# microsoft/ConfigNet

Measured on AMD Instinct MI355X. Metric: train-step images/sec at 256x256 (G+D fwd+bwd), higher is better.
Workload: dtype f32; 1 GPU; ConfigNet second-stage iteration (D + synth-D + latent-D + G + EMA), 256x256, batch 16 per GPU, fp32, Keras-Adam; global_batch=16, resolution=256, latent_dim=145, parallelism=dp1, losses_finite=True

## Files before the change

### confignet_amd/_lib.py

```python
import ctypes
import os

_HERE = os.path.dirname(os.path.abspath(__file__))
LIB_PATH = os.environ.get("CN_LIB") or os.path.join(_HERE, "libconfignet_hip.so")


class CnSumJob(ctypes.Structure):
    _fields_ = [("src", ctypes.c_void_p), ("dst", ctypes.c_void_p), ("count", ctypes.c_longlong), ("parts", ctypes.c_int),
                ("accumulate", ctypes.c_int)]


class CnDepthJob(ctypes.Structure):
    _fields_ = [("a", ctypes.c_void_p), ("b", ctypes.c_void_p), ("c", ctypes.c_void_p), ("m", ctypes.c_int), ("n", ctypes.c_int),
                ("k", ctypes.c_int), ("lda", ctypes.c_int), ("ldb", ctypes.c_int), ("ldc", ctypes.c_int)]


class CnRowsJob(ctypes.Structure):
    _fields_ = [("a", ctypes.c_void_p), ("b", ctypes.c_void_p), ("c", ctypes.c_void_p), ("bias", ctypes.c_void_p), ("mask", ctypes.c_void_p)] + \
               [(n_, ctypes.c_int) for n_ in ("m", "n", "k", "lda", "ldb", "ldc", "tb", "act", "accumulate")] + [("slope", ctypes.c_float)]


class CnGanJob(ctypes.Structure):
    _fields_ = [("s", ctypes.c_void_p), ("out", ctypes.c_void_p), ("gout", ctypes.c_void_p), ("n", ctypes.c_int), ("label", ctypes.c_float)]

# ... 56 lines not shown
    "cn_gemm_rows_grouped": [_p, _i, _p],
    "cn_gemm_rows_grouped_k": [_p, _i, _p],
    "cn_gemm_rows_grouped_plan": [_p, _i, ctypes.POINTER(_i), _i, ctypes.POINTER(_i)],
    "cn_conv_tune": [_i, _i, ctypes.c_long],
    "cn_conv_fwd_plan": [_G, _i, _i, _i, _i, _i, _i, _i, ctypes.POINTER(ctypes.c_int * 8)],
    "cn_conv_fwd_plan_ep": [_G, _i, _i, _i, _i, _i, _i, _i, _i, ctypes.POINTER(ctypes.c_int * 8)],
    "cn_conv_loop_select": [_i, _i, _i, _i],
    "cn_fwd2_col_block": [_i, _i, _i, _i, _i, _i],
    "cn_conv_fwd_dt": [_p, _p, _i, _p, _p, _p, _i, _i, _f, _p],
    "cn_conv_dgrad_dt": [_p, _p, _i, _p, _p, _i, _p],
    "cn_conv_wgrad_c3_partials": [],
    "cn_conv_wgrad_c3": [_p, _p, _p, _i, _p, _p, _i, _p],
    "cn_conv_wino_filter": [_p, _p, _i, _i, _i, _p],
    "cn_conv_fwd_wino": [_i, _i, _i, _i, _i, _p, _p, _p, _p, _i, _f, _p],
    "cn_conv_fwd_wino_ep": [_i, _i, _i, _i, _i, _p, _p, _p, _p, _p, _p, _p],
    "cn_conv_fwd_wino4": [_i, _i, _i, _i, _i, _p, _p, _p, _p, _i, _f, _p],
    "cn_conv_fwd_wino4_ep": [_i, _i, _i, _i, _i, _p, _p, _p, _p, _i, _f, _i, _p, _p, _p, _p, _i, _f, _p],
    "cn_conv_wino4_filter": [_p, _p, _i, _i, _i, _p],
    "cn_sumpool2": [_p, _p, _i, _i, _i, _i, _i, _i, _i, _p],
    "cn_gemm": [_i, _i, _i, _i, _i, _p, _i, _p, _i, _p, _i, _p, _i, _f, _p],
    "cn_gemm_plan": [_i] * 10 + [ctypes.POINTER(ctypes.c_int * 9)],
    "cn_nc_reduce4": [_p, _p, _i, _i, _i, _f, _i, _i, _p],
    "cn_nc_reduce": [_p, _p, _p, _p, _i, _i, _i, _i, _f, _i, _p],
    "cn_nc_reduce_plan": [_i, _i, _i, _i, _i, _i, ctypes.POINTER(ctypes.c_int * 8)],
    "cn_nc_lin2": [_p, _p, _p, _p, _p, _p, _p, _p, _i, _i, _i, _i, _i, _f, _i, _p],
    "cn_nc_rows_plan": [ctypes.c_longlong, _i, _i, ctypes.POINTER(ctypes.c_int * 2)],
    "cn_norm_coef_fwd": [_i, _p, _p, _p, _p, _p, _p, _p, _p, _i, _i, _i, _f, _p, _i, _p],
    "cn_norm_coef_bwd": [_i, _p, _p, _p, _p, _p, _p, _p, _p, _p, _p, _i, _i, _i, _f, _p],
    "cn_dual_tail_coef_fwd": [_p] * 13 + [_i, _i, _i, _f, _i, _i, _p],
    "cn_dual_tail_coef_bwd": [_p] * 13 + [ctypes.POINTER(ctypes.c_void_p), _i, _i, _i, _f, _i, _i, _p],
    "cn_dual_tail_gx": [_p] * 12 + [_i, _i, _i, _f, _i, _i, _p],
    "cn_dual_tail_gx_tx": [_p] * 18 + [_i, _i, _i, _f, _i, _i, _i, _p],
    "cn_norm_apply": [_i, _i] + [_p] * 13 + [_i, _i, _i, _f, _i, _f, _i, _p],
    "cn_nc_reduce_hxt": [_p, _p, _p, _p, _i, _i, _i, _f, _i, _i, _i, _p],
    "cn_zero": [_p, ctypes.c_size_t, _p],
    "cn_set_deterministic": [_i],
    "cn_get_deterministic": [],
    "cn_det_release_stream": [_p],
    "cn_gemm_acc": [_i, _i, _i, _i, _i, _p, _i, _p, _i, _p, _i, _p],
    "cn_sum_rows_into": [_p, _p, _i, _i, _i, _p],
    "cn_bn_act_bwd": [_p, _p, _p, _p, _p, _p, _p, _p, _i, _i, _i, _i, _i, _i, _p],
    "cn_nc_reduce_dact": [_p, _p, _p, _p, _p, _i, _i, _i, _i, _f, _i, _i, _p],
    "cn_act_fwd": [_p, _p, _z, _i, _f, _i, _p],
    "cn_act_bwd": [_p, _p, _p, _z, _i, _f, _i, _p],
    "cn_act_bwd_bias": [_p, _p, _p, _p, _i, _i, _i, _i, _f, _i, _i, _p],
    "cn_axpby": [_p, _p, _p, _z, _f, _f, _i, _p],
    "cn_mul": [_p, _p, _p, _z, _i, _p],
    "cn_sqdiff_sum": [_p, _p, _p, _z, _f, _i, _p],
    "cn_row_sumsq": [_p, _p, _i, _z, _p],
    "cn_row_scale": [_p, _p, _p, _i, _z, _f, _i, _p],
    "cn_row_scale_diff": [_p, _p, _p, _p, _i, ctypes.c_size_t, _f, _i, _p],
    "cn_tap_bwd": [_p, _p, _p, _p, _p, _i, ctypes.c_size_t, _f, _i, _f, _i, _p],
    "cn_maxpool2_bwd_act": [_p, _p, _p, _p, _f, _p, _i, _i, _i, _i, _i, _i, _p],
    "cn_stream_plan": [_i, _i, ctypes.c_longlong, _z, _i, _i, _i, _i, _i, _i, ctypes.c_uint, _i, ctypes.POINTER(ctypes.c_longlong * 4)],
    "cn_stream_plan_ptrs": [_i, _i, _i, ctypes.c_longlong, _z, _i, _i, _i, _i, _i, _i, ctypes.POINTER(ctypes.c_void_p * 4), _i, ctypes.POINTER(ctypes.c_longlong * 4)],
    "cn_stream_last_plan": [ctypes.POINTER(ctypes.c_longlong * 5)],
    "cn_masked_diff": [_p, _p, _p, _p, _z, _i, _p],
    "cn_maxpool_fwd": [_p, _p, _i, _i, _i, _i, _i, _i, _i, _i, _p],
    "cn_maxpool_bwd": [_p, _p, _p, _i, _i, _i, _i, _i, _i, _i, _i, _p],
    "cn_avgpool3_same": [_p, _p, _i, _i, _i, _i, _i, _p],
    "cn_dwconv3x3_fwd": [_p, _p, _p, _p, _i, _i, _i, _i, _i, _i, _f, _p],
    "cn_image_preprocess": [_p, _i, _p, _i, _i, _i, _i, _i, _i, _f, _f, _p],
    "cn_dwconv3x3_dgrad": [_p, _p, _p, _i, _i, _i, _i, _i, _p],
    "cn_dwconv3x3_wgrad_slices": [_i, _i, _i, _i, _i],
    "cn_dwconv3x3_wgrad": [_p, _p, _p, _i, _i, _i, _i, _i, _i, _p],
    "cn_bn_train_coef": [_p] * 12 + [ctypes.c_longlong, _i, _f, ctypes.c_double, _i, _p],
# ... 51 lines not shown
```

### confignet_amd/csrc/elementwise.hip

```cpp
#include "common.h"
#include "typed.h"
#include <stdlib.h>

namespace {

__device__ __forceinline__ float lrelu(float v, float s) { return v > 0.f ? v : v * s; }


template <int V> struct RowV { float v[V]; };

template <int V, typename T>
__device__ __forceinline__ RowV<V> ld_row(const T* p) {
    RowV<V> r;
    if constexpr (V == 4) {
        const float4 t = ld4<T>(p);
        r.v[0] = t.x; r.v[1] = t.y; r.v[2] = t.z; r.v[3] = t.w;
    } else {
        r.v[0] = ldf<T>(p);
    }
    return r;
}
template <int V, typename T>
__device__ __forceinline__ void st_row(T* p, const RowV<V>& r) {
    if constexpr (V == 4) st4<T>(p, make_float4(r.v[0], r.v[1], r.v[2], r.v[3]));
// ... 1208 lines not shown
    }
    CN_DISPATCH_DT(dt, {
        if (V == 4) hipLaunchKernelGGL((nc_lin2_kernel<4, T>), dim3(ew_blocks(total)), dim3(256), 0, st, (const T*)x1, a1, (const T*)x2, a2, bb, a3, b3, (T*)y, total, s, c, cstride, flags, slope, period2);
        else hipLaunchKernelGGL((nc_lin2_kernel<1, T>), dim3(ew_blocks(total)), dim3(256), 0, st, (const T*)x1, a1, (const T*)x2, a2, bb, a3, b3, (T*)y, total, s, c, cstride, flags, slope, period2);
    });
    CN_LAUNCH_CHECK();
    return CN_OK;
}

extern "C" int cn_norm_apply(int mode, int dir, const void* x1, const void* x2, const float* sa, const float* sb, const float* p1,
                             const float* p2, float* save_mean, float* save_r, float* gp1, float* gp2, const float* a3,
                             const float* b3, void* y, int n, int s, int c, float eps, int flags, float slope, int dt, void* stream) {
    CN_CHECK_ARG((mode == 0 || mode == 1) && (dir == 0 || dir == 1) && x1 && sa && sb && p1 && save_mean && save_r && y && n > 0 && s > 0 && c > 0 &&
                 (dt == CN_F32 || dt == CN_BF16), "norm_apply: bad args");
    CN_CHECK_ARG(mode == 0 || dir == 1 || p2, "norm_apply: instance norm needs beta");
    CN_CHECK_ARG(dir == 0 || (x2 && gp1 && (mode == 0 || gp2)), "norm_apply: backward needs x and the parameter gradients' tensors");
    if (c % 4 != 0) return CN_EUNSUPPORTED;
    const int period2 = flags >> 8;
    CN_CHECK_ARG(period2 == 0 || (x2 && n % period2 == 0), "norm_apply: bad x2 period %d for n = %d", period2, n);
    flags &= 255;
    const int CG = c / 4;
    const long G = (long)s * CG;
    const NcRowsPlan rp = plan_nc_rows(G, CG, n);
    if (!rp.rows || (long)rp.gx * 256 < CG) return CN_EUNSUPPORTED;
    NormApplyArgs A;
    A.mode = mode; A.dir = dir; A.N = n; A.C = c; A.invS = 1.f / (float)s; A.eps = eps;
    A.s1 = sa; A.s2 = sb; A.p1 = p1; A.p2 = p2; A.sm = save_mean; A.sr = save_r; A.gp1 = gp1; A.gp2 = gp2;
    CN_DISPATCH_DT(dt, hipLaunchKernelGGL((norm_apply_rows_kernel<T>), dim3(rp.gx, n), dim3(256), 0, (hipStream_t)stream, A, (const T*)x1,
                                          (const T*)x2, a3, b3, (T*)y, (int)G, CG, flags, slope, period2));
    CN_LAUNCH_CHECK();
    return CN_OK;
}

#define EW_LAUNCH(kernel, n, ...)                                                                              \
    hipLaunchKernelGGL(kernel, dim3(ew_blocks(n)), dim3(256), 0, (hipStream_t)stream, __VA_ARGS__);             \
    CN_LAUNCH_CHECK();                                                                                         \
    return CN_OK;

static inline bool alv(const void* p, int dt) { return ((uintptr_t)p & (dt == CN_BF16 ? 7 : 15)) == 0; }
struct StreamPtrs { const void* p[4]; };
static inline unsigned stream_mask(int op, int dt, int dst_dt, const StreamPtrs& o) {
    unsigned m = 0;
    for (int i = 0; i < SP_OPERANDS[op]; ++i)
        if (alv(o.p[i], op == SP_CAST && i == 1 ? dst_dt : dt)) m |= 1u << i;
    return m;
}
static inline StreamReq stream_req(int op, int dt, long rows, size_t row) {
    return StreamReq{op, dt, rows, row, 0, 0, 0, 0, 0, 0, 0u, cn_det()};
}
static inline StreamReq pool_req(int op, int dt, int n, int h, int w, int c, int k, int s, int pad) {
    return StreamReq{op, dt, n, 0, c, h, w, k, s, pad, 0u, cn_det()};
}
static thread_local long long g_stream_last[5] = {-1, 0, 0, 0, 0};
static inline int stream_entry_plan(StreamReq r, int dst_dt, const StreamPtrs& o, StreamPlan* sp) {
    r.aligned = stream_mask(r.op, r.dt, dst_dt, o);
    const int e = plan_stream(r, sp);
    g_stream_last[0] = e ? -1 : r.op; g_stream_last[1] = sp->path; g_stream_last[2] = sp->gx; g_stream_last[3] = sp->gy; g_stream_last[4] = sp->parts;
    return e;
}
#define EW_LAUNCH_VT(kernel, op, n, ptrs, dt, ...)                                                                                \
    CN_CHECK_ARG((dt) == CN_F32 || (dt) == CN_BF16, "bad dtype code %d", (int)(dt));                                                \
    StreamPlan sp;                                                                                                                \
    if (int e__ = stream_entry_plan(stream_req(op, dt, 1, n), dt, ptrs, &sp)) return e__;                                         \
    CN_DISPATCH_DT(dt, {                                                                                                          \
        if (sp.path == SP_VEC) hipLaunchKernelGGL((kernel<true, T>), dim3(sp.gx), dim3(256), 0, (hipStream_t)stream, __VA_ARGS__); \
        else hipLaunchKernelGGL((kernel<false, T>), dim3(sp.gx), dim3(256), 0, (hipStream_t)stream, __VA_ARGS__);                  \
    });                                                                                                                           \
// ... 437 lines not shown
```

### confignet_amd/functional.py

```python
import contextlib

import torch
from torch.autograd import Function

from . import ops
from .ops import ACT_LRELU, ACT_NONE, ACT_RELU, ACT_TANH, ConvSpec

_INPUT_GRADS_ONLY = False
FUSED_TAIL_STATS = True
FUSED_R1_TAIL = True
BN_BWD_FUSED = True


@contextlib.contextmanager
def input_grads_only():
    global _INPUT_GRADS_ONLY
    prev, _INPUT_GRADS_ONLY = _INPUT_GRADS_ONLY, True
    try:
        yield
    finally:
        _INPUT_GRADS_ONLY = prev


class _RefuseFn(Function):
# ... 416 lines not shown
        if x1 is not None and ctx.needs_input_grad[0]:
            gx1 = NcLinFn.apply(gy, a1, None, None, None, pc)
        if a1 is not None and ctx.needs_input_grad[1]:
            sum_gy, ga1 = NcSumDotFn.apply(gy, x1, pc)
        if x2 is not None and ctx.needs_input_grad[2]:
            gx2 = NcLinFn.apply(gy, a2, None, None, None, pc)
        if a2 is not None and ctx.needs_input_grad[3]:
            sum_gy2, ga2 = NcSumDotFn.apply(gy, x2, pc)
            sum_gy = sum_gy if sum_gy is not None else sum_gy2
        if need_b:
            gb = sum_gy if sum_gy is not None else NcSumDotFn.apply(gy, None, pc)[0]
        return gx1, ga1, gx2, ga2, gb, None, None


def nc_stats(x, per_channel=False):
    return NcSumDotFn.apply(x, None, per_channel)


def nc_lin(x1, a1=None, x2=None, a2=None, b=None, per_channel=False):
    return NcLinFn.apply(x1, a1, x2, a2, b, per_channel)


def _spatial(x):
    return x.numel() // (x.shape[0] * x.shape[-1])


class AdaInFn(Function):

    @staticmethod
    def forward(ctx, x, scale_bias):
        x, sb = _cg(x), _cg(scale_bias)
        sp = _spatial(x)
        st = ops.take_stats(x, "act")
        s1, s2 = st if st is not None else ops.nc_reduce(x)
        fused = ops.norm_apply_fwd(ops.NORM_ADAIN, x, s1, s2, sb, None, 1e-3)
        if fused is not None:
            y, mean, r = fused
            ctx.save_for_backward(x, sb, mean, r)
            return y
        a, b, mean, r = ops.norm_coef_fwd(ops.NORM_ADAIN, s1, s2, sb, None, sp, 1e-3, x)
        ctx.save_for_backward(x, sb, mean, r)
        return ops.nc_lin2(tuple(x.shape), x, a, b=b)

    @staticmethod
    def backward(ctx, gy):
        if torch.is_grad_enabled():
            raise RuntimeError("AdaInFn is first-order only; use adain_composite()")
        x, sb, mean, r = ctx.saved_tensors
        gy = _cg(gy)
        t1, t2 = ops.nc_reduce(gy, x)
        fused = ops.norm_apply_bwd(ops.NORM_ADAIN, gy, x, t1, t2, mean, r, sb, 1e-3)
        if fused is not None:
            return fused[0], fused[1]
        c1, c2, c0, gsb, _ = ops.norm_coef_bwd(ops.NORM_ADAIN, t1, t2, mean, r, sb, _spatial(x), 1e-3)
        return ops.nc_lin2(tuple(x.shape), gy, c1, x, c2, c0), gsb


def adain(x, scale_bias):
    return AdaInFn.apply(x, scale_bias)


def adain_composite(x, scale_bias):
    c = x.shape[-1]
    s_, b_ = scale_bias[:, :c], scale_bias[:, c:]
    inv = 1.0 / _spatial(x)
    s1, s2 = nc_stats(x)
    mu = s1 * inv
    var = s2 * inv - mu * mu
    a = torch.rsqrt(var + 1e-3) * (s_ + 1.0)
    return nc_lin(x, a, None, None, b_ - mu * a)


class DiscrTailFn(Function):

    @staticmethod
    def forward(ctx, x, gamma, beta, want_style, slope):
        ctx.set_materialize_grads(False)
        x, gamma, beta = _cg(x), _cg(gamma), _cg(beta)
        sp = _spatial(x)
        style = smean = ssd = None
        st = ops.take_stats(x, "pre4")
        if st is not None:
            s1, s2, a1, a2 = st
            if want_style:
                style, _, smean, ssd = ops.norm_coef_fwd(ops.NORM_STYLE, s1, s2, None, None, sp, 1e-6)
        elif want_style and FUSED_TAIL_STATS and x.shape[-1] % 4 == 0:
            s1, s2, a1, a2 = ops.nc_reduce4(x, slope)
            style, _, smean, ssd = ops.norm_coef_fwd(ops.NORM_STYLE, s1, s2, None, None, sp, 1e-6)
        else:
            if want_style:
                s1, s2 = ops.nc_reduce(x)
                style, _, smean, ssd = ops.norm_coef_fwd(ops.NORM_STYLE, s1, s2, None, None, sp, 1e-6)
            a1, a2 = ops.nc_reduce(x, flags=1, slope=slope)
        fused = ops.norm_apply_fwd(ops.NORM_INSTANCE, x, a1, a2, gamma, beta, 1e-3, flags=1, slope=slope)
        if fused is not None:
            y, mean, q = fused
        else:
            a, b, mean, q = ops.norm_coef_fwd(ops.NORM_INSTANCE, a1, a2, gamma, beta, sp, 1e-3)
            y = ops.nc_lin2(tuple(x.shape), x, a, b=b, flags=1, slope=slope)
        ctx.save_for_backward(x, gamma, mean, q, smean, ssd)
        ctx.slope, ctx.want_style = slope, want_style
        nd = [t for t in (mean, q, smean, ssd) if t is not None]
        ctx.mark_non_differentiable(*nd)
        return y, style, mean, q, smean, ssd

    @staticmethod
    def backward(ctx, gy, gstyle, *_):
        if torch.is_grad_enabled():
            raise RuntimeError("DiscrTailFn is first-order only; use the composite discr_block path")
        x, gamma, mean, q, smean, ssd = ctx.saved_tensors
        sp = _spatial(x)
        have_y = gy is not None
        d2 = d0 = None
        if ctx.want_style and gstyle is not None:
            _, d2, d0, _, _ = ops.norm_coef_bwd(ops.NORM_STYLE, _cg(gstyle), None, smean, ssd, None, sp, 1e-6)
        if have_y:
            gy = _cg(gy)
            t1, t2 = ops.nc_reduce(gy, x, flags=2, slope=ctx.slope)
            fused = ops.norm_apply_bwd(ops.NORM_INSTANCE, gy, x, t1, t2, mean, q, gamma, 1e-3, flags=2 | 4, slope=ctx.slope, a3=d2, b3=d0)
            if fused is not None:
                return fused[0], fused[1], fused[2], None, None
            c1, c2, c0, ggamma, gbeta = ops.norm_coef_bwd(ops.NORM_INSTANCE, t1, t2, mean, q, gamma, sp, 1e-3)
            gx = ops.nc_lin2(tuple(x.shape), gy, c1, x, c2, c0, flags=2 | 4, slope=ctx.slope, a3=d2, b3=d0)
            return gx, ggamma, gbeta, None, None
        gx = ops.nc_lin2(tuple(x.shape), x, d2, b=d0) if d2 is not None else torch.zeros_like(x)
        return gx, torch.zeros_like(gamma), torch.zeros_like(gamma), None, None


class DualTailFn(Function):

    @staticmethod
    def forward(ctx, tx, x, gamma, mean, q, smean, ssd, want_ty, want_style, slope):
        ctx.set_materialize_grads(False)
        tx, x = _cg(tx), _cg(x)
        sp = _spatial(x)
        shape = tuple(x.shape)
        ta = T = U = None
        if want_ty:
            ta = ops.act_bwd(tx, x, ACT_LRELU, slope)
            T = ops.nc_reduce(ta, x, flags=2, slope=slope)
        if want_style:
            U = ops.nc_reduce(tx, x)
        C1, C2, C0, tstyle = ops.dual_tail_coef_fwd(T, U, mean if want_ty else None, q if want_ty else None,
                                                    smean if want_style else None, ssd if want_style else None,
                                                    gamma, sp)
        ty = ops.nc_lin2(shape, ta, C1, x, C2, C0, flags=2, slope=slope) if want_ty else None
        ctx.save_for_backward(tx, x, gamma, mean, q, smean, ssd, ta,
                              T[0] if T else None, T[1] if T else None, U[0] if U else None, U[1] if U else None)
        ctx.cfg = (want_ty, want_style, slope)
        return ty, tstyle

    @staticmethod
    def backward(ctx, h, u):
        if torch.is_grad_enabled():
            raise RuntimeError("DualTailFn is first-order only")
        tx, x, gamma, mean, q, smean, ssd, ta, T1, T2, U1, U2 = ctx.saved_tensors
        want_ty, want_style, slope = ctx.cfg
# ... 357 lines not shown
```

### confignet_amd/ops.py

```python
import contextlib
import ctypes
import math
import os
import threading

import torch

from ._lib import CN_BF16, CN_EUNSUPPORTED, CN_F32, CN_U8, CnConvGeom, CnDepthJob, CnGanJob, CnRowsJob, CnSumJob, check, lib

ACT_NONE, ACT_LRELU, ACT_RELU, ACT_TANH, ACT_RELU6, ACT_SIGMOID = 0, 1, 2, 3, 4, 5

ACT_DTYPE = torch.float32


def set_activation_dtype(dtype):
    global ACT_DTYPE
    if isinstance(dtype, str):
        dtype = {"f32": torch.float32, "fp32": torch.float32, "float32": torch.float32, "bf16": torch.bfloat16,
                 "bfloat16": torch.bfloat16}[dtype]
    assert dtype in (torch.float32, torch.bfloat16)
    ACT_DTYPE = dtype


def _stream():
# ... 944 lines not shown
    n, s, c = _nsc(x)
    y = torch.empty_like(x)
    mean = torch.empty((n, c), device=x.device, dtype=torch.float32)
    r = torch.empty_like(mean)
    rc = lib.cn_norm_apply(mode, 0, _ptr(x), None, _fptr(s1), _fptr(s2), _fptr(_c(p1)), _fptr(None if p2 is None else _c(p2)), _ptr(mean), _ptr(r),
                           None, None, None, None, _ptr(y), n, s, c, eps, flags, slope, _dt(x), _stream())
    if rc == CN_EUNSUPPORTED:
        return None
    check(rc, "cn_norm_apply")
    return y, mean, r


def norm_apply_bwd(mode, gy, x, t1, t2, mean, r, p1, eps, flags=0, slope=0.0, a3=None, b3=None):
    if not NORM_APPLY or x.shape[-1] % 4 or x.dtype != torch.float32 or gy.dtype != torch.float32:
        return None
    gy, x = _unify(gy, x)
    n, s, c = _nsc(x)
    if flags & 4:
        _log_mask(x)
    gx = torch.empty_like(x)
    if mode == NORM_ADAIN:
        gp1, gp2 = torch.empty((n, 2 * c), device=x.device, dtype=torch.float32), None
    else:
        gp1 = torch.empty((c,), device=x.device, dtype=torch.float32)
        gp2 = torch.empty_like(gp1)
    rc = lib.cn_norm_apply(mode, 1, _ptr(gy), _ptr(x), _fptr(t1), _fptr(t2), _fptr(_c(p1)), None, _ptr(mean), _ptr(r), _ptr(gp1), _ptr(gp2),
                           _fptr(a3), _fptr(b3), _ptr(gx), n, s, c, eps, flags, slope, _dt(x), _stream())
    if rc == CN_EUNSUPPORTED:
        return None
    check(rc, "cn_norm_apply")
    return gx, gp1, gp2


def dual_tail_coef_fwd(T, U, mean, q, sm, ssd, gamma, spatial, eps=1e-3):
    ref = mean if mean is not None else sm
    period, c = ref.shape
    mk = lambda *sh: torch.empty(sh, device=ref.device, dtype=torch.float32)
    C1 = C2 = C0 = ts = None
    n_inst = n_style = 0
    if T is not None:
        n_inst = T[0].shape[0]
        C1, C2, C0 = mk(n_inst, c), mk(n_inst, c), mk(n_inst, c)
    if U is not None:
        n_style = U[0].shape[0]
        ts = mk(n_style, 2 * c)
    T1, T2 = T if T is not None else (None, None)
    U1, U2 = U if U is not None else (None, None)
    check(lib.cn_dual_tail_coef_fwd(_ptr(T1), _ptr(T2), _ptr(U1), _ptr(U2), _ptr(mean), _ptr(q), _ptr(sm), _ptr(ssd),
                                    _ptr(gamma), _ptr(C1), _ptr(C2), _ptr(C0), _ptr(ts), n_inst + n_style, c, spatial, eps,
                                    n_style, period, _stream()),
          "cn_dual_tail_coef_fwd")
    return C1, C2, C0, ts


def dual_tail_coef_bwd(H, E, u, T, U, mean, q, sm, ssd, gamma, spatial, eps=1e-3):
    ref = mean if mean is not None else sm
    period, c = ref.shape
    names = ["K1", "K2", "K0", "D2", "D0", "kh", "kt", "ka", "kc", "et", "ex", "e0", "ggamma", "ggamma_rows"]
    out = {k: None for k in names}
    mk = lambda *sh: torch.empty(sh, device=ref.device, dtype=torch.float32)
    n_inst = n_style = 0
    if H is not None:
        n_inst = H[0].shape[0]
        for k in ("K1", "K2", "K0", "kh", "kt", "ka", "kc", "ggamma_rows"):
            out[k] = mk(n_inst, c)
        out["ggamma"] = mk(c)
# ... 623 lines not shown
```

### include/confignet_hip.h

```cpp
#ifndef CONFIGNET_HIP_H
#define CONFIGNET_HIP_H
#include <stddef.h>
#include <stdint.h>

#ifdef __cplusplus
extern "C" {
#endif

#define CN_OK 0
#define CN_EINVAL (-1)
#define CN_EHIP (-2)
#define CN_EUNSUPPORTED (-3)

#define CN_F32 0
#define CN_BF16 1
#define CN_U8 2

#define CN_ACT_NONE 0
#define CN_ACT_LRELU 1
#define CN_ACT_RELU 2
#define CN_ACT_TANH 3
#define CN_ACT_RELU6 4
#define CN_ACT_SIGMOID 5

// ... 121 lines not shown
int cn_gemm_plan(int trans_a, int trans_b, int m, int n, int k, int ldc, int has_bias, int act, int accumulate, int deterministic,
                 int out[9]);

int cn_set_deterministic(int on);
int cn_get_deterministic(void);
int cn_det_release_stream(void* stream);
int cn_zero(void* p, size_t bytes, void* stream);
int cn_gemm_acc(int trans_a, int trans_b, int m, int n, int k, const float* a, int lda, const float* b, int ldb,
                float* c, int ldc, void* stream);
int cn_sum_rows_into(const float* src, float* dst, int rows, int cols, int accumulate, void* stream);

int cn_nc_reduce_plan(int n, int s, int c, int nsums, int prezeroed, int det, int out[8]);
int cn_nc_reduce4(const void* x, float* out, int n, int s, int c, float slope, int flags, int dt, void* stream);
int cn_nc_reduce(const void* x1, const void* x2, float* sum1, float* sum2, int n, int s, int c,
                 int flags, float slope, int dt, void* stream);
int cn_nc_reduce_dact(const void* x1, const void* x2, float* sum1, float* sum2, void* dact_out, int n, int s, int c,
                      int flags, float slope, int act, int dt, void* stream);
int cn_bn_act_bwd(const void* gy, const void* y, const void* x, const float* a, void* g_out, void* gx, float* sum_g,
                  float* sum_gx, int n, int s, int c, int act, int flags, int dt, void* stream);
int cn_nc_lin2(const void* x1, const float* a1, const void* x2, const float* a2, const float* bb,
               const float* a3, const float* b3, void* y, int n, int s, int c, int cstride, int flags,
               float slope, int dt, void* stream);
int cn_nc_rows_plan(long long G, int CG, int ny, int out[2]);

int cn_norm_coef_fwd(int mode, const float* s1, const float* s2, const float* p1, const float* p2, float* A,
                     float* B, float* save_mean, float* save_r, int n, int c, int S, float eps, const void* x, int dt,
                     void* stream);
int cn_norm_coef_bwd(int mode, const float* t1, const float* t2, const float* save_mean, const float* save_r,
                     const float* p1, float* c1, float* c2, float* c0, float* gp1, float* gp2, int n, int c,
                     int S, float eps, void* stream);
int cn_norm_apply(int mode, int dir, const void* x1, const void* x2, const float* sa, const float* sb, const float* p1,
                  const float* p2, float* save_mean, float* save_r, float* gp1, float* gp2, const float* a3, const float* b3,
                  void* y, int n, int s, int c, float eps, int flags, float slope, int dt, void* stream);

int cn_dual_tail_coef_fwd(const float* T1, const float* T2, const float* U1, const float* U2, const float* mean,
                          const float* q, const float* sm, const float* ssd, const float* gamma, float* C1,
                          float* C2, float* C0, float* tstyle, int n, int c, int S, float eps, int n_style, int period,
                          void* stream);
int cn_dual_tail_coef_bwd(const float* H1, const float* H2p, const float* E, const float* u, const float* T1,
                          const float* T2, const float* U1, const float* U2, const float* mean, const float* q,
                          const float* sm, const float* ssd, const float* gamma, float* const* out13, int n, int c,
                          int S, float eps, int n_style, int period, void* stream);
int cn_dual_tail_gx(const void* h, const void* ta, const void* tx, const void* x, const float* kh,
                    const float* kt, const float* ka, const float* kc, const float* et, const float* ex,
                    const float* e0, void* out, int n, int s, int c, float slope, int nrep, int dt, void* stream);
int cn_dual_tail_gx_tx(const void* h, const void* ta, const void* tx, const void* x, const float* kh, const float* kt,
                       const float* ka, const float* kc, const float* et, const float* ex, const float* e0,
                       const float* K1, const float* K2, const float* K0, const float* D2, const float* D0, void* out,
                       void* out_tx, int n, int s, int c, float slope, int nrep, int ta_is_tx, int dt, void* stream);
int cn_nc_reduce_hxt(const void* h, const void* x, const void* ta, float* out, int n, int s, int c, float slope, int period,
                     int flags, int dt, void* stream);

int cn_act_fwd(const void* x, void* y, size_t numel, int act, float slope, int dt, void* stream);
int cn_act_bwd(const void* gy, const void* y, void* gx, size_t numel, int act, float slope, int dt, void* stream);
int cn_act_bwd_bias(const void* gy, const void* y, void* gx, float* gb, int n, int s, int c, int act, float slope, int flags,
                    int dt, void* stream);
int cn_axpby(const void* x, const void* y, void* out, size_t numel, float a, float b, int dt, void* stream);
int cn_mul(const void* x, const void* y, void* out, size_t numel, int dt, void* stream);
int cn_sqdiff_sum(const void* a, const void* b, float* out, size_t numel, float scale, int dt, void* stream);
int cn_row_sumsq(const float* x, float* out, int n, size_t row, void* stream);
int cn_row_scale(const void* x, const float* s, void* out, int n, size_t row, float k, int dt, void* stream);
int cn_row_scale_diff(const void* x, const void* x2, const float* s, void* out, int n, size_t row, float k, int dt, void* stream);
int cn_tap_bwd(const void* y, const void* target, const void* g, const float* s, void* out, int n, size_t row, float k,
               int act, float slope, int dt, void* stream);
int cn_maxpool2_bwd_act(const void* x, const void* gy, const void* target, const float* s, float k, void* gx, int n, int h,
                        int w, int c, int s_rows, int dt, void* stream);
// ... 75 lines not shown
```

Before: 449.7 images/sec.

## Fuse norm statistics reduction and apply into one single-pass kernel for small spatial sizes

Adds a norm_one kernel that loads each (sample, channel-group) slab into registers, reduces the statistics in shared memory, computes the coefficients and writes the normalized output in one launch. It covers AdaIN and instance-norm forward and backward, including the style and LeakyReLU variants. It replaces the separate nc_reduce plus norm_apply launches and the second read of x when the spatial size is at most 1024. It only applies to f32 in non-deterministic mode, and the per-block register tiling limits it to small spatial sizes; larger layers fall back to the old path.

```diff
diff --git a/confignet_amd/_lib.py b/confignet_amd/_lib.py
--- a/confignet_amd/_lib.py
+++ b/confignet_amd/_lib.py
@@ -112,6 +112,8 @@
     "cn_dual_tail_gx": [_p] * 12 + [_i, _i, _i, _f, _i, _i, _p],
     "cn_dual_tail_gx_tx": [_p] * 18 + [_i, _i, _i, _f, _i, _i, _i, _p],
     "cn_norm_apply": [_i, _i] + [_p] * 13 + [_i, _i, _i, _f, _i, _f, _i, _p],
+    "cn_norm_one": [_i, _i] + [_p] * 14 + [_i, _i, _i, _f, _f, _f, _i, _p],
+    "cn_norm_one_plan": [_i, _i, _i, _i, _i, ctypes.POINTER(ctypes.c_int * 6)],
     "cn_nc_reduce_hxt": [_p, _p, _p, _p, _i, _i, _i, _f, _i, _i, _i, _p],
     "cn_zero": [_p, ctypes.c_size_t, _p],
     "cn_set_deterministic": [_i],
diff --git a/confignet_amd/csrc/elementwise.hip b/confignet_amd/csrc/elementwise.hip
--- a/confignet_amd/csrc/elementwise.hip
+++ b/confignet_amd/csrc/elementwise.hip
@@ -1264,7 +1264,267 @@
     return CN_OK;
 }
 
-#define EW_LAUNCH(kernel, n, ...)                                                                              \
+namespace {
+
+struct NormOneArgs {
+    int S, C;
+    float invS, eps, eps_style, slope;
+    const float* p1; const float* p2;
+    float* sm; float* sr;
+    float* style; float* smean; float* ssd;
+    const float* gstyle;
+    float* g1; float* g2;
+    float* sums;
+};
+
+template <int Q>
+__device__ __forceinline__ void norm_one_sum(float (&acc)[Q][4], float4 (*red)[256], float4 (*red2)[256]) {
+    const int tx = threadIdx.x, ty = threadIdx.y, TX = blockDim.x, TY = blockDim.y;
+#pragma unroll
+    for (int q = 0; q < Q; ++q) red[q][ty * TX + tx] = make_float4(acc[q][0], acc[q][1], acc[q][2], acc[q][3]);
+    __syncthreads();
+    const int J = TY < 16 ? TY : 16, chunk = TY / J;
+    float4 (*src)[256] = red;
+    if (chunk > 1) {
+        if (ty < J) {
+#pragma unroll
+            for (int q = 0; q < Q; ++q) {
+                float4 t = make_float4(0.f, 0.f, 0.f, 0.f);
+                for (int y = ty * chunk; y < (ty + 1) * chunk; ++y) {
+                    const float4 v = red[q][y * TX + tx];
+                    t.x += v.x; t.y += v.y; t.z += v.z; t.w += v.w;
+                }
+                red2[q][ty * TX + tx] = t;
+            }
+        }
+        __syncthreads();
+        src = red2;
+    }
+#pragma unroll
+    for (int q = 0; q < Q; ++q) {
+        float4 t = make_float4(0.f, 0.f, 0.f, 0.f);
+        for (int j = 0; j < J; ++j) {
+            const float4 v = src[q][j * TX + tx];
+            t.x += v.x; t.y += v.y; t.z += v.z; t.w += v.w;
+        }
+        acc[q][0] = t.x; acc[q][1] = t.y; acc[q][2] = t.z; acc[q][3] = t.w;
+    }
+}
+
+template <int MODE, int DIR, int VPT>
+__global__ __launch_bounds__(256) void norm_one_kernel(NormOneArgs A, const float* __restrict__ x1, const float* __restrict__ x2,
+                                                       float* __restrict__ y) {
+    constexpr int Q = (MODE == 1 && DIR == 0) ? 4 : 2;
+    __shared__ float4 red[Q][256];
+    __shared__ float4 red2[Q][256];
+    const int tx = threadIdx.x, ty = threadIdx.y, TX = blockDim.x, TY = blockDim.y;
+    const int S = A.S, C = A.C;
+    const int cg = blockIdx.x * TX + tx, n = blockIdx.y, N = gridDim.y;
+    const bool live = cg * 4 < C;
+    const long base = (long)n * S * C + (long)cg * 4;
+    const float slope = A.slope;
+    const bool have1 = DIR == 0 || x1 != nullptr;
+    const float* xp = DIR == 0 ? x1 : x2;
+    RowV<4> a[VPT], b[VPT];
+#pragma unroll
+    for (int u = 0; u < VPT; ++u) {
+        const int s = ty + u * TY;
+        const bool in = live && s < S;
+#pragma unroll
+        for (int e = 0; e < 4; ++e) { a[u].v[e] = 0.f; b[u].v[e] = 0.f; }
+        if (in && have1) a[u] = ld_row<4, float>(x1 + base + (long)s * C);
+        if (DIR == 1 && in) b[u] = ld_row<4, float>(x2 + base + (long)s * C);
+    }
+    float acc[Q][4];
+#pragma unroll
+    for (int q = 0; q < Q; ++q)
+#pragma unroll
+        for (int e = 0; e < 4; ++e) acc[q][e] = 0.f;
+    if (have1) {
+#pragma unroll
+        for (int u = 0; u < VPT; ++u)
+#pragma unroll
+            for (int e = 0; e < 4; ++e) {
+                const float v = a[u].v[e];
+                if (DIR == 0 && MODE == 0) {
+                    acc[0][e] += v;
+                    acc[1][e] += v * v;
+                } else if (DIR == 0) {
+                    const float l = lrelu(v, slope);
+                    acc[0][e] += v;
+                    acc[1][e] += v * v;
+                    acc[2][e] += l;
+                    acc[3][e] += l * l;
+                } else {
+                    const float w = MODE == 1 ? lrelu(b[u].v[e], slope) : b[u].v[e];
+                    acc[0][e] += v;
+                    acc[1][e] += v * w;
+                }
+            }
+        norm_one_sum<Q>(acc, red, red2);
+    }
+    const bool side = live && ty == 0;
+    float k1[4], k2[4], kb[4], k3[4], kb3[4];
+#pragma unroll
+    for (int e = 0; e < 4; ++e) {
+        k1[e] = k2[e] = kb[e] = k3[e] = kb3[e] = 0.f;
+        if (!live) continue;
+        const int c = cg * 4 + e;
+        const long i = (long)n * C + c;
+        if (side && A.sums && have1) {
+#pragma unroll
+            for (int q = 0; q < Q; ++q) A.sums[((long)q * N + n) * C + c] = acc[q][e];
+        }
+        if (DIR == 0) {
+            if (MODE == 1 && A.style) {
+                const float m = acc[0][e] * A.invS;
+                const float var = fmaxf(acc[1][e] * A.invS - m * m, 0.f);
+                const float sd = sqrtf(var + A.eps_style);
+                if (side) {
+                    A.smean[i] = m; A.ssd[i] = sd;
+                    A.style[(long)n * 2 * C + c] = m; A.style[(long)n * 2 * C + C + c] = sd;
+                }
+            }
+            const float s1 = acc[MODE == 1 ? 2 : 0][e], s2 = acc[MODE == 1 ? 3 : 1][e];
+            const float mu = s1 * A.invS;
+            float var = fmaxf(s2 * A.invS - mu * mu, 0.f);
+            float rr, k;
+            if (MODE == 0) {
+                if (cn_adain_refine(mu, var, A.eps)) var = cn_var_two_pass<float>(xp + (long)n * S * C + c, S, C, mu, A.invS);
+                rr = rsqrtf(var + A.eps);
+                k = rr * (A.p1[(long)n * 2 * C + c] + 1.f);
+                kb[e] = A.p1[(long)n * 2 * C + C + c] - mu * k;
+            } else {
+                rr = 1.f / (sqrtf(var) + A.eps);
+                k = A.p1[c] * rr;
+                kb[e] = A.p2[c] - mu * k;
+            }
+            k1[e] = k;
+            if (side) { A.sm[i] = mu; A.sr[i] = rr; }
+        } else {
+            if (have1) {
+                const float mu = A.sm[i], t1 = acc[0][e], t2 = acc[1][e];
+                if (MODE == 0) {
+                    const float r = A.sr[i], sp1 = A.p1[(long)n * 2 * C + c] + 1.f;
+                    const float gs = r * (t2 - mu * t1);
+                    const float q1 = r * sp1;
+                    const float q2 = -r * r * sp1 * gs * A.invS;
+                    k1[e] = q1; k2[e] = q2;
+                    kb[e] = -q1 * t1 * A.invS - q2 * mu;
+                    if (side) { A.g1[(long)n * 2 * C + c] = gs; A.g1[(long)n * 2 * C + C + c] = t1; }
+                } else {
+                    const float q = A.sr[i], gam = A.p1[c];
+                    const float sigma = fmaxf(1.f / q - A.eps, 1e-20f);
+                    const float Gm = gam * (t2 - mu * t1);
+                    const float q1 = q * gam;
+                    const float q2 = -q * q * Gm * A.invS / sigma;
+                    k1[e] = q1; k2[e] = q2;
+                    kb[e] = -q1 * t1 * A.invS - q2 * mu;
+                    if (side && A.g1) { A.g1[i] = q * (t2 - mu * t1); A.g2[i] = t1; }
+                }
+            }
+            if (MODE == 1 && A.gstyle) {
+                const float sd = A.ssd[i];
+                const float gmu = A.gstyle[(long)n * 2 * C + c], gsd = A.gstyle[(long)n * 2 * C + C + c];
+                k3[e] = gsd * A.invS / sd;
+                kb3[e] = gmu * A.invS - k3[e] * A.smean[i];
+            }
+        }
+    }
+    if (!live) return;
+#pragma unroll
+    for (int u = 0; u < VPT; ++u) {
+        const int s = ty + u * TY;
+        if (s >= S) break;
+        RowV<4> r;
+#pragma unroll
+        for (int e = 0; e < 4; ++e) {
+            if (DIR == 0) {
+                r.v[e] = kb[e] + k1[e] * (MODE == 1 ? lrelu(a[u].v[e], slope) : a[u].v[e]);
+            } else {
+                const float xv = b[u].v[e];
+                float t = kb[e];
+                t += k1[e] * a[u].v[e];
+                t += k2[e] * (MODE == 1 ? lrelu(xv, slope) : xv);
+                if (MODE == 1) {
+                    t *= xv > 0.f ? 1.f : slope;
+                    t += k3[e] * xv + kb3[e];
+                }
+                r.v[e] = t;
+            }
+        }
+        st_row<4, float>(y + base + (long)s * C, r);
+    }
+}
+
+}
+
+struct NormOnePlan { int ok, CW, TX, TY, VPT, cblk; };
+static NormOnePlan plan_norm_one(int mode, int dir, int n, int s, int c) {
+    NormOnePlan p = {0, 0, 0, 0, 0, 0};
+    if (mode < 0 || mode > 1 || dir < 0 || dir > 1 || n < 1 || n > 65535 || s < 1 || s > 1024 || c < 4 || c % 4 != 0) return p;
+    const int cw_min = c >= 8 ? 8 : 4;
+    for (int cw = 64; cw >= cw_min; cw >>= 1) {
+        const int TX = cw / 4, TY = 256 / TX;
+        int vpt = 1;
+        while (vpt * TY < s) vpt <<= 1;
+        if (vpt > 8) continue;
+        p.ok = 1; p.CW = cw; p.TX = TX; p.TY = TY; p.VPT = vpt; p.cblk = cn_cdiv(c, cw);
+        if ((long)n * p.cblk >= 256) break;
+    }
+    return p;
+}
+
+extern "C" int cn_norm_one_plan(int mode, int dir, int n, int s, int c, int out[6]) {
+    CN_CHECK_ARG(out, "norm_one_plan: NULL");
+    const NormOnePlan p = plan_norm_one(mode, dir, n, s, c);
+    const int v[6] = {p.ok, p.CW, p.TX, p.TY, p.VPT, p.cblk};
+    for (int i = 0; i < 6; ++i) out[i] = v[i];
+    return CN_OK;
+}
+
+extern "C" int cn_norm_one(int mode, int dir, const void* x1, const void* x2, const float* p1, const float* p2, float* save_mean,
+                           float* save_r, float* style, float* smean, float* ssd, const float* gstyle, float* g1, float* g2,
+                           float* sums_out, void* y, int n, int s, int c, float eps, float eps_style, float slope, int dt, void* stream) {
+    CN_CHECK_ARG((mode == 0 || mode == 1) && (dir == 0 || dir == 1) && y && p1 && n > 0 && s > 0 && c > 0, "norm_one: bad args");
+    if (dir == 0) {
+        CN_CHECK_ARG(x1 && save_mean && save_r && (mode == 0 || p2), "norm_one: forward needs x, mean, r (and beta)");
+        CN_CHECK_ARG(!style || (mode == 1 && smean && ssd), "norm_one: style needs mode 1, smean and ssd");
+    } else {
+        CN_CHECK_ARG(x2 && (x1 || (mode == 1 && gstyle)), "norm_one: backward needs x and a cotangent");
+        CN_CHECK_ARG(!x1 || (save_mean && save_r), "norm_one: backward needs mean and r");
+        CN_CHECK_ARG(mode == 1 || g1, "norm_one: AdaIN backward needs d[s|b]");
+        CN_CHECK_ARG(mode == 0 || ((g1 == nullptr) == (g2 == nullptr)), "norm_one: d gamma and d beta come together");
+        CN_CHECK_ARG(!gstyle || (mode == 1 && smean && ssd), "norm_one: d style needs mode 1, smean and ssd");
+    }
+    if (dt != CN_F32) return CN_EUNSUPPORTED;
+    const NormOnePlan p = plan_norm_one(mode, dir, n, s, c);
+    if (!p.ok) return CN_EUNSUPPORTED;
+    for (const void* q : {x1, x2, (const void*)y})
+        if ((uintptr_t)q & 15) return CN_EUNSUPPORTED;
+    NormOneArgs A;
+    A.S = s; A.C = c; A.invS = 1.f / (float)s; A.eps = eps; A.eps_style = eps_style; A.slope = slope;
+    A.p1 = p1; A.p2 = p2; A.sm = save_mean; A.sr = save_r; A.style = style; A.smean = smean; A.ssd = ssd; A.gstyle = gstyle;
+    A.g1 = g1; A.g2 = g2; A.sums = sums_out;
+    hipStream_t st = (hipStream_t)stream;
+    const dim3 grid(p.cblk, n), block(p.TX, p.TY);
+#define NORM_ONE_VPT(M, D)                                                                                                                  \
+    switch (p.VPT) {                                                                                                                        \
+        case 1: hipLaunchKernelGGL((norm_one_kernel<M, D, 1>), grid, block, 0, st, A, (const float*)x1, (const float*)x2, (float*)y); break; \
+        case 2: hipLaunchKernelGGL((norm_one_kernel<M, D, 2>), grid, block, 0, st, A, (const float*)x1, (const float*)x2, (float*)y); break; \
+        case 4: hipLaunchKernelGGL((norm_one_kernel<M, D, 4>), grid, block, 0, st, A, (const float*)x1, (const float*)x2, (float*)y); break; \
+        default: hipLaunchKernelGGL((norm_one_kernel<M, D, 8>), grid, block, 0, st, A, (const float*)x1, (const float*)x2, (float*)y); break; \
+    }
+    if (mode == 0 && dir == 0) { NORM_ONE_VPT(0, 0) }
+    else if (mode == 0) { NORM_ONE_VPT(0, 1) }
+    else if (dir == 0) { NORM_ONE_VPT(1, 0) }
+    else { NORM_ONE_VPT(1, 1) }
+#undef NORM_ONE_VPT
+    CN_LAUNCH_CHECK();
+    return CN_OK;
+}
+
+#define EW_LAUNCH(kernel, n, ...)                                                                             \
     hipLaunchKernelGGL(kernel, dim3(ew_blocks(n)), dim3(256), 0, (hipStream_t)stream, __VA_ARGS__);             \
     CN_LAUNCH_CHECK();                                                                                         \
     return CN_OK;
diff --git a/confignet_amd/functional.py b/confignet_amd/functional.py
--- a/confignet_amd/functional.py
+++ b/confignet_amd/functional.py
@@ -472,12 +472,19 @@
         x, sb = _cg(x), _cg(scale_bias)
         sp = _spatial(x)
         st = ops.take_stats(x, "act")
-        s1, s2 = st if st is not None else ops.nc_reduce(x)
-        fused = ops.norm_apply_fwd(ops.NORM_ADAIN, x, s1, s2, sb, None, 1e-3)
+        fused = ops.norm_one_fwd(ops.NORM_ADAIN, x, sb, None, 1e-3) if st is None else None
+        if fused is not None:
+            ops._norm_log("one", 0, x, ops.NORM_ADAIN)
+        else:
+            s1, s2 = st if st is not None else ops.nc_reduce(x)
+            fused = ops.norm_apply_fwd(ops.NORM_ADAIN, x, s1, s2, sb, None, 1e-3)
+            if fused is not None:
+                ops._norm_log("apply", 0, x, ops.NORM_ADAIN)
         if fused is not None:
             y, mean, r = fused
             ctx.save_for_backward(x, sb, mean, r)
             return y
+        ops._norm_log("lin2", 0, x, ops.NORM_ADAIN)
         a, b, mean, r = ops.norm_coef_fwd(ops.NORM_ADAIN, s1, s2, sb, None, sp, 1e-3, x)
         ctx.save_for_backward(x, sb, mean, r)
         return ops.nc_lin2(tuple(x.shape), x, a, b=b)
@@ -488,10 +495,16 @@
             raise RuntimeError("AdaInFn is first-order only; use adain_composite()")
         x, sb, mean, r = ctx.saved_tensors
         gy = _cg(gy)
+        fused = ops.norm_one_bwd(ops.NORM_ADAIN, gy, x, sb, mean, r, 1e-3)
+        if fused is not None:
+            ops._norm_log("one", 1, x, ops.NORM_ADAIN)
+            return fused[0], fused[1]
         t1, t2 = ops.nc_reduce(gy, x)
         fused = ops.norm_apply_bwd(ops.NORM_ADAIN, gy, x, t1, t2, mean, r, sb, 1e-3)
         if fused is not None:
+            ops._norm_log("apply", 1, x, ops.NORM_ADAIN)
             return fused[0], fused[1]
+        ops._norm_log("lin2", 1, x, ops.NORM_ADAIN)
         c1, c2, c0, gsb, _ = ops.norm_coef_bwd(ops.NORM_ADAIN, t1, t2, mean, r, sb, _spatial(x), 1e-3)
         return ops.nc_lin2(tuple(x.shape), gy, c1, x, c2, c0), gsb
 
@@ -520,6 +533,15 @@
         sp = _spatial(x)
         style = smean = ssd = None
         st = ops.take_stats(x, "pre4")
+        ctx.slope, ctx.want_style = slope, want_style
+        ctx.beta_ref = beta if beta.requires_grad else None
+        one = ops.norm_one_fwd(ops.NORM_INSTANCE, x, gamma, beta, 1e-3, slope, want_style) if st is None else None
+        if one is not None:
+            ops._norm_log("one", 0, x, ops.NORM_INSTANCE)
+            y, mean, q, style, smean, ssd = one
+            ctx.save_for_backward(x, gamma, mean, q, smean, ssd)
+            ctx.mark_non_differentiable(*[t for t in (mean, q, smean, ssd) if t is not None])
+            return y, style, mean, q, smean, ssd
         if st is not None:
             s1, s2, a1, a2 = st
             if want_style:
@@ -534,12 +556,13 @@
             a1, a2 = ops.nc_reduce(x, flags=1, slope=slope)
         fused = ops.norm_apply_fwd(ops.NORM_INSTANCE, x, a1, a2, gamma, beta, 1e-3, flags=1, slope=slope)
         if fused is not None:
+            ops._norm_log("apply", 0, x, ops.NORM_INSTANCE)
             y, mean, q = fused
         else:
+            ops._norm_log("lin2", 0, x, ops.NORM_INSTANCE)
             a, b, mean, q = ops.norm_coef_fwd(ops.NORM_INSTANCE, a1, a2, gamma, beta, sp, 1e-3)
             y = ops.nc_lin2(tuple(x.shape), x, a, b=b, flags=1, slope=slope)
         ctx.save_for_backward(x, gamma, mean, q, smean, ssd)
-        ctx.slope, ctx.want_style = slope, want_style
         nd = [t for t in (mean, q, smean, ssd) if t is not None]
         ctx.mark_non_differentiable(*nd)
         return y, style, mean, q, smean, ssd
@@ -551,6 +574,29 @@
         x, gamma, mean, q, smean, ssd = ctx.saved_tensors
         sp = _spatial(x)
         have_y = gy is not None
+        gst = _cg(gstyle) if (ctx.want_style and gstyle is not None) else None
+        if have_y or gst is not None:
+            want_p = (ctx.needs_input_grad[1] or ctx.needs_input_grad[2]) and not _INPUT_GRADS_ONLY
+            one = ops.norm_one_bwd(ops.NORM_INSTANCE, _cg(gy) if have_y else None, x, gamma, mean, q, 1e-3, ctx.slope, gst, smean, ssd,
+                                   want_params=want_p)
+            if one is not None:
+                ops._norm_log("one", 1, x, ops.NORM_INSTANCE)
+                gx, rows_g, rows_b = one
+                if not have_y:
+                    return gx, torch.zeros_like(gamma), torch.zeros_like(gamma), None, None
+                if rows_g is None:
+                    return gx, None, None, None, None
+                grads = []
+                for rows, ref in ((rows_g, gamma), (rows_b, ctx.beta_ref)):
+                    slot = ops.sink_for(ref)
+                    if slot is not None:
+                        ops.sum_rows_into(rows, slot)
+                        grads.append(None)
+                    else:
+                        dst = torch.empty_like(gamma)
+                        ops.sum_rows_into(rows, dst, accumulate=False, defer=False)
+                        grads.append(dst)
+                return gx, grads[0], grads[1], None, None
         d2 = d0 = None
         if ctx.want_style and gstyle is not None:
             _, d2, d0, _, _ = ops.norm_coef_bwd(ops.NORM_STYLE, _cg(gstyle), None, smean, ssd, None, sp, 1e-6)
@@ -559,10 +605,13 @@
             t1, t2 = ops.nc_reduce(gy, x, flags=2, slope=ctx.slope)
             fused = ops.norm_apply_bwd(ops.NORM_INSTANCE, gy, x, t1, t2, mean, q, gamma, 1e-3, flags=2 | 4, slope=ctx.slope, a3=d2, b3=d0)
             if fused is not None:
+                ops._norm_log("apply", 1, x, ops.NORM_INSTANCE)
                 return fused[0], fused[1], fused[2], None, None
+            ops._norm_log("lin2", 1, x, ops.NORM_INSTANCE)
             c1, c2, c0, ggamma, gbeta = ops.norm_coef_bwd(ops.NORM_INSTANCE, t1, t2, mean, q, gamma, sp, 1e-3)
             gx = ops.nc_lin2(tuple(x.shape), gy, c1, x, c2, c0, flags=2 | 4, slope=ctx.slope, a3=d2, b3=d0)
             return gx, ggamma, gbeta, None, None
+        ops._norm_log("lin2", 1, x, ops.NORM_INSTANCE)
         gx = ops.nc_lin2(tuple(x.shape), x, d2, b=d0) if d2 is not None else torch.zeros_like(x)
         return gx, torch.zeros_like(gamma), torch.zeros_like(gamma), None, None
 
diff --git a/confignet_amd/ops.py b/confignet_amd/ops.py
--- a/confignet_amd/ops.py
+++ b/confignet_amd/ops.py
@@ -1000,6 +1000,67 @@
     return gx, gp1, gp2
 
 
+NORM_ONE = True
+NORM_LOG = None
+
+
+def _norm_log(path, dir_, x, mode):
+    if NORM_LOG is not None:
+        NORM_LOG.append((path, dir_, _nsc(x), mode))
+
+
+def norm_one_plan(mode, dir_, n, s, c):
+    out = (ctypes.c_int * 6)()
+    check(lib.cn_norm_one_plan(mode, dir_, n, s, c, ctypes.byref(out)), "cn_norm_one_plan")
+    return list(out)
+
+
+def _norm_one_wanted(*ts):
+    return NORM_ONE and not DETERMINISTIC and all(t is None or t.dtype == torch.float32 for t in ts)
+
+
+def norm_one_fwd(mode, x, p1, p2, eps, slope=0.0, want_style=False, eps_style=1e-6, sums=None):
+    n, s, c = _nsc(x)
+    if not _norm_one_wanted(x) or not norm_one_plan(mode, 0, n, s, c)[0]:
+        return None
+    dev = x.device
+    y = torch.empty_like(x)
+    mean = torch.empty((n, c), device=dev, dtype=torch.float32)
+    r = torch.empty_like(mean)
+    style = smean = ssd = None
+    if want_style:
+        style = torch.empty((n, 2 * c), device=dev, dtype=torch.float32)
+        smean, ssd = torch.empty_like(mean), torch.empty_like(mean)
+    rc = lib.cn_norm_one(mode, 0, _ptr(x), None, _fptr(_c(p1)), _fptr(None if p2 is None else _c(p2)), _ptr(mean), _ptr(r), _ptr(style),
+                         _ptr(smean), _ptr(ssd), None, None, None, _fptr(sums), _ptr(y), n, s, c, eps, eps_style, slope, _dt(x), _stream())
+    if rc == CN_EUNSUPPORTED:
+        return None
+    check(rc, "cn_norm_one")
+    return (y, mean, r) if mode == NORM_ADAIN else (y, mean, r, style, smean, ssd)
+
+
+def norm_one_bwd(mode, gy, x, p1, mean, r, eps, slope=0.0, gstyle=None, smean=None, ssd=None, want_params=True, sums=None):
+    n, s, c = _nsc(x)
+    if not _norm_one_wanted(gy, x) or not norm_one_plan(mode, 1, n, s, c)[0]:
+        return None
+    gx = torch.empty_like(x)
+    g1 = g2 = None
+    if mode == NORM_ADAIN:
+        g1 = torch.empty((n, 2 * c), device=x.device, dtype=torch.float32)
+    elif want_params and gy is not None:
+        g1 = torch.empty((n, c), device=x.device, dtype=torch.float32)
+        g2 = torch.empty_like(g1)
+    rc = lib.cn_norm_one(mode, 1, _ptr(gy), _ptr(x), _fptr(_c(p1)), None, _fptr(mean), _fptr(r), None, _fptr(smean), _fptr(ssd),
+                         _fptr(None if gstyle is None else _c(gstyle)), _ptr(g1), _ptr(g2), _fptr(sums), _ptr(gx), n, s, c, eps, 1e-6,
+                         slope, _dt(x), _stream())
+    if rc == CN_EUNSUPPORTED:
+        return None
+    check(rc, "cn_norm_one")
+    if mode == NORM_INSTANCE and gy is not None:
+        _log_mask(x)
+    return gx, g1, g2
+
+
 def dual_tail_coef_fwd(T, U, mean, q, sm, ssd, gamma, spatial, eps=1e-3):
     ref = mean if mean is not None else sm
     period, c = ref.shape
diff --git a/include/confignet_hip.h b/include/confignet_hip.h
--- a/include/confignet_hip.h
+++ b/include/confignet_hip.h
@@ -177,6 +177,10 @@
 int cn_norm_apply(int mode, int dir, const void* x1, const void* x2, const float* sa, const float* sb, const float* p1,
                   const float* p2, float* save_mean, float* save_r, float* gp1, float* gp2, const float* a3, const float* b3,
                   void* y, int n, int s, int c, float eps, int flags, float slope, int dt, void* stream);
+int cn_norm_one(int mode, int dir, const void* x1, const void* x2, const float* p1, const float* p2, float* save_mean,
+                float* save_r, float* style, float* smean, float* ssd, const float* gstyle, float* g1, float* g2,
+                float* sums_out, void* y, int n, int s, int c, float eps, float eps_style, float slope, int dt, void* stream);
+int cn_norm_one_plan(int mode, int dir, int n, int s, int c, int out[6]);
 
 int cn_dual_tail_coef_fwd(const float* T1, const float* T2, const float* U1, const float* U2, const float* mean,
                           const float* q, const float* sm, const float* ssd, const float* gamma, float* C1,
```

Result: no change. 450.8 images/sec, median of 5 (+0.3%).
